# Plachtaa/FAcodec

Measured on NVIDIA H100. Metric: audio_seconds_per_second, higher is better.
Workload: dtype f32 I/O and accumulation; every product is a 3-MMA split of fp32 operands: fp16 hi + 2^11-scaled fp16 lo (22 mantissa bits, register-promoted accumulation) upstream of the VQ, bf16 hi + bf16 lo (16 bits) downstream

## Files before the change

### facodec_b200/_lib.py

```python
import ctypes
import os

from . import build as _build

_c = ctypes
_LIB = None


class FacError(RuntimeError):
    pass


def lib_path():
    return _build.LIB


def load():
    global _LIB
    if _LIB is not None:
        return _LIB
    path = lib_path()
    if not os.path.exists(path):
        raise FacError(f"{path} not found: build it with `python -m facodec_b200.build` "
                       "(needs nvcc; there is no CPU fallback)")
    L = ctypes.CDLL(path)
    vp, i32, i64p, fp = _c.c_void_p, _c.c_int, _c.c_void_p, _c.c_void_p
    sigs = {
        "fac_abi_version": ([], i32),
        "fac_create": ([_c.POINTER(vp), i32], i32),
        "fac_destroy": ([vp], i32),
        "fac_last_error": ([vp], _c.c_char_p),
        "fac_load_tensor": ([vp, i32, _c.c_char_p, fp, _c.POINTER(_c.c_int64), i32], i32),
        "fac_finalize": ([vp], i32),
        "fac_encode": ([vp, fp, i32, i32, fp, vp], i32),
        "fac_encode_frames": ([i32], i32),
        "fac_quantize": ([vp, fp, fp, i32, i32, i32, i32, fp, i32, i64p, fp, fp, fp, fp, fp, fp, i64p, i64p, i64p, vp], i32),
        "fac_decode": ([vp, fp, i32, i32, fp, vp], i32),
        "fac_codec_forward": ([vp, fp, i32, i32, i32, fp, i64p, i64p, i64p, fp, vp], i32),
        "fac_codec_forward_host": ([vp, fp, i32, i32, i32, fp, i64p, i64p, i64p, vp], i32),
        "fac_codec_encode": ([vp, fp, i32, i32, i32, i64p, i64p, i64p, fp, vp], i32),
        "fac_dequantize": ([vp, i64p, i64p, i32, i64p, i32, fp, i32, i32, fp, fp, fp, fp, vp], i32),
        "fac_codes_decode": ([vp, i64p, i64p, i32, i64p, i32, fp, i32, i32, fp, vp], i32),
        "fac_redecode": ([vp, i64p, i64p, i32, fp, i32, i32, i32, i32, i32, fp, vp], i32),
        "fac_redecoder_decode": ([vp, fp, i32, i32, fp, vp], i32),
        "fac_voice_convert": ([vp, i64p, i64p, i32, fp, i32, i32, i32, i32, i32, fp, vp], i32),
        "fac_dataset_mel": ([vp, fp, i32, i32, fp, vp], i32),
        "fac_head_begin": ([vp], i32),
        "fac_head_tensor": ([vp, i32, _c.c_char_p, fp, _c.POINTER(_c.c_int64), i32], i32),
        "fac_head_finalize": ([vp, i32, i32, i32, i32, i32], i32),
        "fac_head_forward": ([vp, i32, fp, i32, i32, _c.POINTER(vp), vp], i32),
        "fac_rvq_create": ([vp, i32] + [_c.POINTER(vp)] * 5, i32),
        "fac_rvq_destroy": ([vp, i32], i32),
        "fac_stream_begin": ([vp, i32], i32),
        "fac_stream_encode": ([vp, i32, fp, i32, fp, vp], i32),
        "fac_stream_decode": ([vp, i32, fp, i32, fp, vp], i32),
        "fac_stream_decode_codes": ([vp, i32, i64p, i64p, i32, i64p, i32, fp, i32, fp, vp], i32),
        "fac_stream_encode_codes": ([vp, i32, fp, i32, i32, i64p, i64p, i64p, vp], i32),
        "fac_stream_finish_codes": ([vp, i32, i64p, i64p, i64p, fp, vp], i32),
        "fac_stream_end": ([vp, i32], i32),
        "fac_spectral_loss": ([vp, fp, fp, i32, i32, i32, i32, _c.POINTER(_c.c_int), _c.POINTER(_c.c_int), fp, fp,
                               _c.c_float, _c.c_float, _c.c_float, _c.c_float, fp, vp], i32),
        "fac_l1_loss": ([vp, fp, fp, _c.c_longlong, fp, vp], i32),
        "fac_add3": ([vp, fp, fp, fp, _c.c_longlong, fp, vp], i32),
        "fac_reconstruction_loss": ([vp, fp, fp, i32, i32, fp, fp, vp], i32),
        "fac_rvq_forward": ([vp, i32, fp, i32, i32, i32, fp, i64p, fp, vp], i32),
        "fac_alias_free_act": ([vp, fp, i32, i32, i32, i32, fp, fp, fp, vp], i32),
        "fac_debug_conv": ([vp, fp, fp, fp] + [i32] * 10 + [fp, fp, i32, fp, fp, i32, vp], i32),
        "fac_debug_conv_tc": ([vp, fp, fp, fp] + [i32] * 10 + [fp, fp, i32, fp, fp, i32, i32, vp], i32),
        "fac_debug_resunit": ([vp, fp, fp, fp, fp, fp, fp, fp, i32, i32, i32, i32, i32, fp, vp], i32),
        "fac_debug_tc_phase_clocks": ([vp, _c.POINTER(_c.c_longlong)], i32),
        "fac_debug_tc_producer_clocks": ([vp, _c.POINTER(_c.c_longlong)], i32),
        "fac_debug_tc_trace": ([vp, _c.POINTER(_c.c_longlong)], i32),
        "fac_debug_lstm_pack": ([fp, i32, i32, fp, _c.c_longlong, _c.POINTER(_c.c_int)], _c.c_longlong),
        "fac_debug_convtr_pack": ([fp, i32, i32, i32, i32, fp, _c.c_longlong], _c.c_longlong),
        "fac_debug_pad_map": ([i32, i32, i32, i32, _c.POINTER(_c.c_int), i32], i32),
        "fac_debug_tc_plan": ([i32] * 8 + [_c.POINTER(_c.c_int)], i32),
        "fac_debug_tc_pack": ([fp, i32, i32, i32, i32, i32, fp, _c.c_longlong], _c.c_longlong),
        "fac_debug_lstm_phase_clocks": ([vp, _c.POINTER(_c.c_longlong)], i32),
        "fac_set_option": ([vp, _c.c_char_p, i32], i32),
        "fac_debug_slstm": ([vp, fp, _c.POINTER(vp), i32, i32, i32, fp, vp], i32),
        "fac_debug_fa_quantize": ([vp, fp, fp, _c.POINTER(vp), fp, i32, i32, i32, i32, i32, fp, fp, fp, fp, i64p, i64p, i64p,
                                   fp, fp, vp], i32),
        "fac_debug_attention": ([vp, fp, fp, fp, fp, i32, i32, i32, _c.c_void_p, i32, vp], i32),
        "fac_debug_tap": ([vp, _c.c_char_p, fp, _c.c_size_t], i32),
        "fac_profile_enable": ([vp, i32], i32),
        "fac_profile_reset": ([vp], i32),
        "fac_profile_get": ([vp, _c.c_char_p, _c.POINTER(_c.c_double), _c.POINTER(_c.c_double),
                             _c.POINTER(_c.c_double), _c.POINTER(_c.c_longlong)], i32),
        "fac_profile_dump": ([vp, _c.c_char_p, _c.c_size_t], _c.c_size_t),
        "fac_workspace_bytes": ([vp], _c.c_size_t),
        "fac_last_launch_count": ([vp], i32),
    }
    for name, (args, res) in sigs.items():
        fn = getattr(L, name)
        fn.argtypes = args
        fn.restype = res
    _LIB = L
    return L


EXPORTED = ["fac_abi_version", "fac_create", "fac_destroy", "fac_last_error", "fac_load_tensor", "fac_finalize",
            "fac_encode", "fac_encode_frames", "fac_quantize", "fac_decode", "fac_codec_forward",
            "fac_codec_forward_host", "fac_codec_encode", "fac_dequantize", "fac_codes_decode", "fac_redecode", "fac_redecoder_decode", "fac_voice_convert", "fac_dataset_mel", "fac_reconstruction_loss", "fac_spectral_loss", "fac_l1_loss", "fac_head_begin", "fac_head_tensor", "fac_head_finalize", "fac_head_forward", "fac_add3", "fac_stream_begin", "fac_stream_encode", "fac_stream_decode", "fac_stream_decode_codes", "fac_stream_encode_codes", "fac_stream_finish_codes", "fac_stream_end", "fac_rvq_create", "fac_rvq_destroy", "fac_rvq_forward", "fac_alias_free_act",
            "fac_debug_conv", "fac_debug_conv_tc", "fac_debug_resunit", "fac_debug_tc_phase_clocks", "fac_debug_tc_producer_clocks", "fac_debug_tc_trace", "fac_debug_lstm_pack", "fac_debug_convtr_pack", "fac_debug_pad_map", "fac_debug_tc_plan", "fac_debug_tc_pack", "fac_debug_lstm_phase_clocks", "fac_set_option", "fac_debug_slstm", "fac_debug_fa_quantize", "fac_debug_attention", "fac_debug_tap", "fac_profile_enable", "fac_profile_reset", "fac_profile_get", "fac_profile_dump",
            "fac_workspace_bytes", "fac_last_launch_count"]


def check(handle, rc, what):
    if rc < 0:
        msg = load().fac_last_error(handle)
        raise FacError(f"{what} failed (status {rc}): {msg.decode() if msg else ''}")
    return rc
```

### facodec_b200/csrc/conv_tc.cu

```cuda
#include <cuda_bf16.h>
#include <cuda_fp16.h>

#include <cstring>
#include <mutex>

#include "common.cuh"
#include "conv_tc_common.cuh"
#include "kernels.h"

namespace fac {

namespace {

using namespace tc;

enum Prec { P_TF32 = 0, P_BF16 = 1, P_F16S = 2, P_F16X2 = 3, P_NONE = -1 };

template <int P> struct PrecT {
    static constexpr int KG = P == P_TF32 ? 4 : 2;
    static constexpr int planes = P == P_F16S ? 1 : 2;
    static constexpr int ksteps = P == P_TF32 ? 2 : 1;
    static constexpr int kind = P == P_TF32 ? WG_TF32 : (P == P_BF16 ? WG_BF16 : WG_F16);
};

__host__ __device__ constexpr int prec_kg(int P) { return P == P_TF32 ? 4 : 2; }
__host__ __device__ constexpr int prec_planes(int P) { return P == P_F16S ? 1 : 2; }
__host__ __device__ constexpr uint32_t master_bytes(bool promoted, int nchunk, int promote_every, int ni) {
    return promoted && nchunk > promote_every ? (uint32_t)ni / 2 * 4 * kThreads : 0u;
}

template <int NI>
__device__ __forceinline__ void zero_acc(float (&a)[NI / 2]) {
#pragma unroll
    for (int i = 0; i < NI / 2; ++i) a[i] = 0.f;
}

template <int P, int NI>
__device__ __forceinline__ void mma_pass(float (&acc)[NI / 2], uint32_t a_addr, uint32_t a_lbo, uint32_t b_addr,
                                         uint32_t b_lbo) {
#pragma unroll
    for (int ks = 0; ks < PrecT<P>::ksteps; ++ks)
        wgmma_ss<NI, PrecT<P>::kind>(acc, gdesc(a_addr + ks * 2 * a_lbo, a_lbo, 128), gdesc(b_addr + ks * 2 * b_lbo, b_lbo, 128));
}

struct Tile {
    int row0, col0, nw;
    int warp, lane;
};

template <int NI, int GROUP = NI, typename F>
__device__ __forceinline__ void for_each_pair(const Tile& tl, const float (&acc)[NI / 2], F&& f) {
#pragma unroll
    for (int j = 0; j < NI / 8; ++j) {
        if (j > 0 && (8 * j) % GROUP == 0 && 8 * j >= tl.nw) break;
#pragma unroll
        for (int h = 0; h < 2; ++h) {
            const int row = tl.row0 + 16 * tl.warp + (tl.lane >> 2) + 8 * h;
            const int col = tl.col0 + 8 * j + 2 * (tl.lane & 3);
            f(row, col, acc[4 * j + 2 * h], acc[4 * j + 2 * h + 1]);
        }
    }
}

template <bool FAST>
__device__ __forceinline__ float act_out(int act, float v, float al, float ia) {
    if (act == ACT_SNAKE) return FAST ? fmaf(ia, sin2_mufu(al * v), v) : snake_fast(v, al, ia);
    if (act == ACT_TANH) return tanhf(v);
    if (act == ACT_MISH) return mish_f(v);
    return v;
}

template <int P1, int P2, bool PROMO, int NI, int MINB = 1, bool TT = false>
__global__ void __launch_bounds__(kThreads, MINB) conv_tc_kernel(TcConvParams p) {
    constexpr bool FUSED = P2 != P_NONE;
    static_assert(!TT || (NI == 64 && !FUSED), "transposed tiles: <= 64 channels x 64 time steps per warpgroup");
    static_assert(NI % 16 == 0 && NI <= (PROMO || MINB == 2 ? 64 : (P1 == P_F16S ? 256 : 128)),
                  "accumulator registers: <= 64 / 128 columns (256 in the one-pass fp16 class at one CTA per SM)");
    constexpr bool F16X2 = P1 == P_F16X2;
    constexpr bool DEC = P1 == P_BF16 || P1 == P_F16S;
    using T1 = PrecT<P1>;
    extern __shared__ __align__(1024) uint8_t smem[];
    uint64_t* full = reinterpret_cast<uint64_t*>(smem);

    const int tid = threadIdx.x, wg = tid >> 7;
    const int BM = 64 * p.MT;
    const int N = p.N, NW = p.MT == 2 ? N : N / 2;
    Tile tl;
    tl.row0 = p.MT == 2 ? 64 * wg : 0;
    tl.col0 = p.MT == 2 ? 0 : wg * NW;
    tl.nw = NW;
    tl.warp = (tid >> 5) & 3;
    tl.lane = tid & 31;
    const int t0 = blockIdx.x * BM, ntile = blockIdx.y, b = blockIdx.z;
    const int Kr = p.Kr, dil = p.dil, Rpad = p.Rpad, nchunk = p.nchunk, S = p.stagesB;
    const int R = BM + (Kr - 1) * dil;
    const uint32_t a_plane = (uint32_t)T1::KG * Rpad * 16, a_bytes = a_plane * T1::planes;
    uint8_t* abuf = smem + kSmemHdr;
    float4* master = reinterpret_cast<float4*>(abuf + 2 * (size_t)a_bytes);
    uint8_t* wbuf = abuf + 2 * (size_t)a_bytes + master_bytes(PROMO, nchunk, p.promote_every, NI);
    uint8_t* a2buf = wbuf + (size_t)S * p.b_slot;
    const uint32_t w_unit1 = (uint32_t)Kr * T1::planes * T1::KG * N * 16;
    const uint32_t w_unit2 = FUSED ? (uint32_t)prec_planes(P2) * prec_kg(P2) * N * 16 : 0;
    const int units = nchunk + (FUSED ? p.nchunk2 : 0);

    if (tid == 0) {
        for (int i = 0; i < S; ++i) mbar_init(&full[i], 1);
        fence_mbar_init();
    }
    __syncthreads();
    auto issue_w = [&](int u) {
        uint64_t* bar = &full[u % S];
        uint8_t* dst = wbuf + (size_t)(u % S) * p.b_slot;
        const uint8_t* src;
        uint32_t bytes;
        if (u < nchunk) { src = reinterpret_cast<const uint8_t*>(p.wblob) + ((size_t)ntile * nchunk + u) * w_unit1; bytes = w_unit1; }
        else { src = reinterpret_cast<const uint8_t*>(p.wblob2) + (size_t)(u - nchunk) * w_unit2; bytes = w_unit2; }
        mbar_arrive_expect_tx(bar, bytes);
        bulk_g2s(dst, src, bytes, bar);
    };
    if (tid == 0)
        for (int u = 0; u < S - 1 && u < units; ++u) issue_w(u);

    const PadMap pm = PadMap::make(p.Tin, p.pad_left_s, p.pad_right_s, p.reflect);
    const float* __restrict__ xb = p.x + (size_t)b * p.x_bstride;
    auto produce = [&](int c) {
        uint8_t* ahi = abuf + (size_t)(c & 1) * a_bytes;
        if constexpr (P1 == P_TF32) produce_chunk<kThreads, false>(p, pm, xb, c, t0, R, Rpad, ahi, ahi + a_plane, tid);
        else if constexpr (P1 == P_BF16) produce_chunk<kThreads, true>(p, pm, xb, c, t0, R, Rpad, ahi, ahi + a_plane, tid);
        else if constexpr (P1 == P_F16S) produce_chunk<kThreads, true, 4, false, false, true>(p, pm, xb, c, t0, R, Rpad, ahi, ahi, tid);
        else produce_chunk<kThreads, false, 4, false, true>(p, pm, xb, c, t0, R, Rpad, ahi, ahi + a_plane, tid);
        fence_proxy_async();
    };
    produce(0);

    float acc[NI / 2];
    float crs[F16X2 ? NI / 2 : 1];
    zero_acc<NI>(acc);
    if constexpr (F16X2) zero_acc<NI>(crs);
    const uint32_t a_lbo = (uint32_t)Rpad * 16, b_lbo = (uint32_t)N * 16;
    const uint32_t abase = smem_u32(abuf), wbase = smem_u32(wbuf), a2base = smem_u32(a2buf);
    const int BM2 = BM;

    auto promote = [&](bool first, bool last) {
        if constexpr (PROMO) {
#pragma unroll
            for (int q = 0; q < NI / 8; ++q) {
                float w[4];
#pragma unroll
                for (int e = 0; e < 4; ++e) {
                    const int i = 4 * q + e;
                    if constexpr (F16X2) { w[e] = acc[i] + crs[i] * kLoUnscale; crs[i] = 0.f; }
                    else w[e] = acc[i];
                }
                float4 m = first ? make_float4(0.f, 0.f, 0.f, 0.f) : master[q * kThreads + tid];
                m.x += w[0]; m.y += w[1]; m.z += w[2]; m.w += w[3];
                if (!last) master[q * kThreads + tid] = m;
                acc[4 * q + 0] = last ? m.x : 0.f;
                acc[4 * q + 1] = last ? m.y : 0.f;
                acc[4 * q + 2] = last ? m.z : 0.f;
                acc[4 * q + 3] = last ? m.w : 0.f;
            }
        }
    };

#pragma unroll 1
    for (int u = 0; u < units; ++u) {
        __syncthreads();
        if (tid == 0 && u + S - 1 < units) issue_w(u + S - 1);
        mbar_wait(&full[u % S], (uint32_t)(u / S) & 1u);
        const uint32_t wslot = wbase + (uint32_t)(u % S) * p.b_slot;
        wg_fence();
        if (u < nchunk) {
            const uint32_t a0 = abase + (uint32_t)(u & 1) * a_bytes + (uint32_t)tl.row0 * 16;
            const uint32_t b0 = wslot + (uint32_t)tl.col0 * 16;
#pragma unroll 1
            for (int tap = 0; tap < Kr; ++tap) {
                const uint32_t ahi = a0 + (uint32_t)(tap * dil) * 16, alo = ahi + a_plane;
                const uint32_t bhi = b0 + (uint32_t)tap * T1::planes * T1::KG * b_lbo, blo = bhi + T1::KG * b_lbo;
                if constexpr (TT) {
                    mma_pass<P1, NI>(acc, bhi, b_lbo, ahi, a_lbo);
                    mma_pass<P1, NI>(crs, bhi, b_lbo, alo, a_lbo);
                    mma_pass<P1, NI>(crs, blo, b_lbo, ahi, a_lbo);
                } else if constexpr (P1 == P_F16S) {
                    mma_pass<P1, NI>(acc, ahi, a_lbo, bhi, b_lbo);
                } else if constexpr (F16X2) {
// ... 81 lines not shown
    for_each_pair<NI>(tl, acc, [&](int row, int col, float v0, float v1) {
        const int t = t0 + row;
        if (t >= p.Tout) return;
        if (bi_p) { const float2 bi = __ldg(reinterpret_cast<const float2*>(bi_p + col)); v0 += bi.x; v1 += bi.y; }
        if (act == ACT_SNAKE) {
            const float2 al = __ldg(reinterpret_cast<const float2*>(al_p + col));
            const float2 ia = __ldg(reinterpret_cast<const float2*>(ia_p + col));
            v0 = act_out<DEC>(ACT_SNAKE, v0, al.x, ia.x);
            v1 = act_out<DEC>(ACT_SNAKE, v1, al.y, ia.y);
        } else if (act != ACT_NONE) {
            v0 = act_out<DEC>(act, v0, 0.f, 0.f);
            v1 = act_out<DEC>(act, v1, 0.f, 0.f);
        }
        if (rb) { const float2 r = *reinterpret_cast<const float2*>(rb + (size_t)t * p.ldy + col); v0 += r.x; v1 += r.y; }
        *reinterpret_cast<float2*>(yb + (size_t)t * p.ldy + col) = make_float2(v0, v1);
    });
}

}

namespace {
constexpr size_t kSmemCap = 227 * 1024;
constexpr size_t kSmemCap2 = 113 * 1024;
int plan_prec(const TcConvParams& p) {
    return p.g1f16 ? P_F16S : (p.f16x2 ? P_F16X2 : (p.bf16 ? P_BF16 : P_TF32));
}
constexpr int f16s_wide_nw(bool fused) { return fused ? 192 : 256; }
}

bool tc_conv_plan(TcConvParams& p) {
    if ((p.Cin % 4) != 0 || ((p.Cin * p.vf) % kChunk) != 0 || (p.Cout % 16) != 0) return false;
    if (p.bf16 && p.promoted) return false;
    if (p.f16x2 && !p.promoted) return false;
    if (p.g1f16 && !p.bf16) return false;
    if (p.tt && !p.f16x2) return false;
    if (p.fused && (p.promoted || p.Cin != p.Cout || p.vf != 1 || p.Cout > 256)) return false;
    const int P1 = plan_prec(p), P2 = p.fused ? (p.bf16 ? P_BF16 : P_TF32) : P_NONE;
    p.nchunk = p.Cin * p.vf / kChunk;
    p.nchunk2 = p.fused ? p.Cout / kChunk : 0;
    p.promote_every = p.promoted ? (p.f16x2 ? (48 / p.Kr < 1 ? 1 : 48 / p.Kr) : (8 / p.Kr < 1 ? 1 : 8 / p.Kr)) : 1;
    const int nw_max = p.promoted ? 64 : 128;
    constexpr size_t kAReserve = 40 * 1024;
    int N = 0;
    for (int cand = p.fused ? p.Cout : 256; cand >= 16 && N == 0; cand -= 16) {
        const bool rows_split = cand <= nw_max, cols_split = (cand / 2) % 16 == 0 && cand / 2 <= nw_max;
        if (p.Cout % cand || !(rows_split || cols_split)) continue;
        size_t slot = (size_t)p.Kr * prec_planes(P1) * prec_kg(P1) * cand * 16, a2 = 0;
        if (P2 != P_NONE) a2 = (size_t)prec_planes(P2) * p.nchunk2 * prec_kg(P2) * 64 * 16;
        if (kSmemHdr + kAReserve + slot + a2 <= kSmemCap) N = cand;
        else if (p.fused) return false;
    }
    if (N == 0) return false;
    struct Layout { int Rpad; size_t slot, total; };
    auto layout = [&](int S, int MT) {
        const int NW = MT == 2 ? N : N / 2, BM = 64 * MT;
        Layout l;
        l.Rpad = BM + (p.Kr - 1) * p.dil;
        while (l.Rpad % 8 != 2) ++l.Rpad;
        const size_t a_bytes = (size_t)prec_planes(P1) * prec_kg(P1) * l.Rpad * 16;
        l.slot = (size_t)p.Kr * prec_planes(P1) * prec_kg(P1) * N * 16;
        size_t a2 = 0;
        if (P2 != P_NONE) {
            const size_t slot2 = (size_t)prec_planes(P2) * prec_kg(P2) * N * 16;
            if (slot2 > l.slot) l.slot = slot2;
            a2 = (size_t)prec_planes(P2) * p.nchunk2 * prec_kg(P2) * BM * 16;
        }
        const size_t master = master_bytes(p.promoted, p.nchunk, p.promote_every, p.tt ? 64 : NW);
        l.total = kSmemHdr + 2 * a_bytes + master + S * l.slot + a2 + (p.tt ? 64 * 16 : 0);
        return l;
    };
    const bool want2 = p.promoted ? !p.tt : (p.occ2_maxn > 0 && N <= p.occ2_maxn);
    for (int two = want2 ? 1 : 0; two >= 0; --two) {
        const size_t cap = two ? kSmemCap2 : kSmemCap;
        const int nwl = two ? 64 : nw_max;
        for (int S = 2; S >= 1; --S)
            for (int MT = 2; MT >= 1; --MT) {
                const int NW = MT == 2 ? N : N / 2;
                const bool wide = !two && P1 == P_F16S && NW == f16s_wide_nw(p.fused);
                if ((NW > nwl && !wide) || NW % 16) continue;
                if (wide && layout(2, 1).total <= kSmemCap2) continue;
                const Layout l = layout(S, MT);
                if (l.total > cap) continue;
                p.N = N; p.MT = MT; p.Rpad = l.Rpad; p.R2pad = 64 * MT; p.stagesB = S; p.b_slot = (int)l.slot;
                p.smem_bytes = l.total;
                p.occ2 = two;
                return true;
            }
    }
    return false;
}

size_t tc_blob_floats(const TcConvParams& p) {
    if (p.g1f16) return (size_t)(p.Cout / p.N) * p.nchunk * p.Kr * 2 * p.N * 4;
    return (size_t)(p.Cout / p.N) * p.nchunk * p.Kr * 2 * ((p.bf16 || p.f16x2) ? 2 : 4) * p.N * 4;
}

static inline uint16_t bf16_rn_host(float f) {
    uint32_t u;
    memcpy(&u, &f, 4);
    u += 0x7FFFu + ((u >> 16) & 1u);
    return (uint16_t)(u >> 16);
}

void tc_pack_blob(const TcConvParams& p, const float* wp, int ldw, float* blob) {
    const int Cw = p.Cin * p.vf;
    if (p.g1f16) {
        uint16_t* ob = reinterpret_cast<uint16_t*>(blob);
        size_t o16 = 0;
        for (int nt = 0; nt < p.Cout / p.N; ++nt)
            for (int c = 0; c < p.nchunk; ++c)
                for (int tap = 0; tap < p.Kr; ++tap)
                    for (int k8 = 0; k8 < 2; ++k8)
                        for (int n = 0; n < p.N; ++n)
                            for (int e = 0; e < 8; ++e) {
                                int kk = tap * Cw + c * tc::kChunk + k8 * 8 + e;
                                __half v = __float2half_rn(wp[(size_t)kk * ldw + nt * p.N + n]);
                                uint16_t bits;
                                memcpy(&bits, &v, 2);
                                ob[o16++] = bits;
                            }
        return;
    }
    if (p.f16x2) {
        uint16_t* ob = reinterpret_cast<uint16_t*>(blob);
        size_t o16 = 0;
        for (int nt = 0; nt < p.Cout / p.N; ++nt)
            for (int c = 0; c < p.nchunk; ++c)
                for (int tap = 0; tap < p.Kr; ++tap)
                    for (int hl = 0; hl < 2; ++hl)
                        for (int k8 = 0; k8 < 2; ++k8)
                            for (int n = 0; n < p.N; ++n)
                                for (int e = 0; e < 8; ++e) {
                                    int kk = tap * Cw + c * tc::kChunk + k8 * 8 + e;
                                    float w = wp[(size_t)kk * ldw + nt * p.N + n];
                                    __half hi = __float2half_rn(w);
                                    __half v = hl == 0 ? hi : __float2half_rn((w - __half2float(hi)) * 2048.0f);
// ... 111 lines not shown
```

### facodec_b200/csrc/conv_tc_common.cuh

```cuda
#pragma once
#include <cuda_bf16.h>
#include <cuda_fp16.h>

#include "common.cuh"
#include "kernels.h"

namespace fac {

namespace tc {

constexpr int kThreads = 256;
constexpr int kChunk = 16;
constexpr int kSmemHdr = 128;

__device__ __forceinline__ uint32_t smem_u32(const void* p) { return (uint32_t)__cvta_generic_to_shared(p); }

__device__ __forceinline__ void mbar_init(uint64_t* bar, uint32_t count) {
    asm volatile("mbarrier.init.shared::cta.b64 [%0], %1;" ::"r"(smem_u32(bar)), "r"(count));
}
__device__ __forceinline__ void mbar_arrive(uint64_t* bar) {
    asm volatile("mbarrier.arrive.shared::cta.b64 _, [%0];" ::"r"(smem_u32(bar)) : "memory");
}
__device__ __forceinline__ void mbar_arrive_expect_tx(uint64_t* bar, uint32_t bytes) {
    asm volatile("mbarrier.arrive.expect_tx.shared::cta.b64 _, [%0], %1;" ::"r"(smem_u32(bar)), "r"(bytes) : "memory");
// ... 156 lines not shown
    uint32_t r;
    asm("cvt.rna.tf32.f32 %0, %1;" : "=r"(r) : "f"(x));
    return __uint_as_float(r);
}


template <bool BF16>
__device__ __forceinline__ void split_store(float4 x4, int pc, int row, int Rpad, uint8_t* ahi, uint8_t* alo) {
    if constexpr (!BF16) {
        float4 hi, lo;
        hi.x = to_tf32(x4.x); lo.x = to_tf32(x4.x - hi.x);
        hi.y = to_tf32(x4.y); lo.y = to_tf32(x4.y - hi.y);
        hi.z = to_tf32(x4.z); lo.z = to_tf32(x4.z - hi.z);
        hi.w = to_tf32(x4.w); lo.w = to_tf32(x4.w - hi.w);
        const size_t off = ((size_t)pc * Rpad + row) * 16;
        *reinterpret_cast<float4*>(ahi + off) = hi;
        *reinterpret_cast<float4*>(alo + off) = lo;
    } else {
        __nv_bfloat162 h01 = __floats2bfloat162_rn(x4.x, x4.y), h23 = __floats2bfloat162_rn(x4.z, x4.w);
        float2 f01 = __bfloat1622float2(h01), f23 = __bfloat1622float2(h23);
        __nv_bfloat162 l01 = __floats2bfloat162_rn(x4.x - f01.x, x4.y - f01.y);
        __nv_bfloat162 l23 = __floats2bfloat162_rn(x4.z - f23.x, x4.w - f23.y);
        const size_t off = ((size_t)(pc >> 1) * Rpad + row) * 16 + (size_t)(pc & 1) * 8;
        uint2 hv, lv;
        hv.x = *reinterpret_cast<uint32_t*>(&h01); hv.y = *reinterpret_cast<uint32_t*>(&h23);
        lv.x = *reinterpret_cast<uint32_t*>(&l01); lv.y = *reinterpret_cast<uint32_t*>(&l23);
        *reinterpret_cast<uint2*>(ahi + off) = hv;
        *reinterpret_cast<uint2*>(alo + off) = lv;
    }
}

constexpr float kLoScale = 2048.0f, kLoUnscale = 1.0f / 2048.0f;
__device__ __forceinline__ void split_store_f16(float4 x4, int pc, int row, int Rpad, uint8_t* ahi, uint8_t* alo) {
    __half2 h01 = __floats2half2_rn(x4.x, x4.y), h23 = __floats2half2_rn(x4.z, x4.w);
    float2 f01 = __half22float2(h01), f23 = __half22float2(h23);
    __half2 l01 = __floats2half2_rn((x4.x - f01.x) * kLoScale, (x4.y - f01.y) * kLoScale);
    __half2 l23 = __floats2half2_rn((x4.z - f23.x) * kLoScale, (x4.w - f23.y) * kLoScale);
    const size_t off = ((size_t)(pc >> 1) * Rpad + row) * 16 + (size_t)(pc & 1) * 8;
    uint2 hv, lv;
    hv.x = *reinterpret_cast<uint32_t*>(&h01); hv.y = *reinterpret_cast<uint32_t*>(&h23);
    lv.x = *reinterpret_cast<uint32_t*>(&l01); lv.y = *reinterpret_cast<uint32_t*>(&l23);
    *reinterpret_cast<uint2*>(ahi + off) = hv;
    *reinterpret_cast<uint2*>(alo + off) = lv;
}

__device__ __forceinline__ void store_f16_single(float4 x4, int pc, int row, int Rpad, uint8_t* ahi) {
    __half2 h01 = __floats2half2_rn(x4.x, x4.y), h23 = __floats2half2_rn(x4.z, x4.w);
    const size_t off = ((size_t)(pc >> 1) * Rpad + row) * 16 + (size_t)(pc & 1) * 8;
    uint2 hv;
    hv.x = *reinterpret_cast<uint32_t*>(&h01); hv.y = *reinterpret_cast<uint32_t*>(&h23);
    *reinterpret_cast<uint2*>(ahi + off) = hv;
}

template <int NT, bool BF16, int BATCH = 4, bool INL = false, bool F16 = false, bool SINGLE = false>
__device__ __forceinline__ void produce_chunk(const TcConvParams& p, const PadMap& pm, const float* __restrict__ xb,
                                              int c, int t0, int R, int Rpad, uint8_t* ahi, uint8_t* alo, int ptid) {
    const int pc = ptid & 3;
    const int j = c * kChunk + pc * 4;
    const int soff = j / p.Cin, ci = j - soff * p.Cin;
    const bool has_alpha = p.in_alpha != nullptr;
    float4 al = make_float4(0.f, 0.f, 0.f, 0.f), ia = al;
    if (has_alpha) {
        al = __ldg(reinterpret_cast<const float4*>(p.in_alpha + ci));
        ia = __ldg(reinterpret_cast<const float4*>(p.in_inv_alpha + ci));
    }
    constexpr int RSTEP = NT / 4;
    const int row_limit = p.Tout + (p.Kr - 1) * p.dil;
    const int vrow0 = t0 - p.PLr;
    const float* __restrict__ xcol = xb + ci;
#pragma unroll 1
    for (int r = ptid >> 2; r < R; r += RSTEP * BATCH) {
        float4 v[BATCH];
#pragma unroll
        for (int u = 0; u < BATCH; ++u) {
            const int rr = r + u * RSTEP;
            v[u] = make_float4(0.f, 0.f, 0.f, 0.f);
            const int vrow = vrow0 + rr;
            if (rr < R && vrow < row_limit) {
                const int src = pm.src(vrow * p.vf + soff);
                if (src >= 0) v[u] = __ldg(reinterpret_cast<const float4*>(xcol + (size_t)src * p.ldx));
            }
        }
#pragma unroll
        for (int u = 0; u < BATCH; ++u) {
            const int rr = r + u * RSTEP;
            if (rr < R) {
                float4 x4 = v[u];
                if (has_alpha) x4 = snake4_sel<BF16, INL>(x4, al, ia);
                if constexpr (SINGLE) store_f16_single(x4, pc, rr, Rpad, ahi);
                else if constexpr (F16) split_store_f16(x4, pc, rr, Rpad, ahi, alo);
                else split_store<BF16>(x4, pc, rr, Rpad, ahi, alo);
            }
        }
    }
}

}

}
```

### facodec_b200/csrc/engine.cu

```cuda
#include <cmath>
#include <cstdio>
#include <cstdlib>
#include <cstring>
#include <map>
#include <string>
#include <vector>

#include "../../include/facodec_b200.h"
#include "../../include/facodec_b200_debug.h"
#include "common.cuh"
#include "kernels.h"

using namespace fac;

namespace {

constexpr int HOP = 300;
constexpr int LATENT = 1024;
constexpr int N_FFT = 2048;
constexpr int WIN = 1200;
constexpr int N_BINS = 1025;
constexpr int SPEC_LD = 2052;
constexpr int SPEC_TC_LD = 2176;
constexpr int N_MELS = 80;
// ... 2564 lines not shown
    for (int i = 0; i < 8; ++i) {
        HostTensor t;
        const bool mat = (i % 4) < 2;
        if (mat) t.shape = {4 * H, H}; else t.shape = {4 * H};
        if (i == 1) t.data.assign(whh_host, whh_host + (size_t)4 * H * H);
        else t.data.assign(t.numel(), 0.f);
        tmp.host[0][std::string("l.") + names[i]] = std::move(t);
    }
    LstmW L;
    try { L = pack_lstm(&tmp, 0, "l"); } catch (const PackError&) { return FAC_ERR_UNSUPPORTED; }
    if (info3) { info3[0] = L.U; info3[1] = L.G; info3[2] = 4 * L.U; }
    if (bf16 == 2 || bf16 == 3) {
        const int p3 = bf16 == 3;
        const long long n2 = (long long)lstm2_pack_words(H, L.U, p3);
        if (!out || capacity_floats < n2) return n2;
        lstm2_pack(whh_host, H, L.U, p3, reinterpret_cast<uint32_t*>(out));
        return n2;
    }
    const long long n = (long long)L.G * H * 4 * L.U;
    if (bf16 && !L.has16) return FAC_ERR_UNSUPPORTED;
    if (!out || capacity_floats < n) return n;
    memcpy(out, tmp.pack.data() + (bf16 ? L.whh16[0] : L.whh[0]), sizeof(float) * (size_t)n);
    return n;
}

long long fac_debug_convtr_pack(const float* w_host, int Cin, int Cout, int stride, int causal, float* out, long long capacity_floats) {
    if (!w_host || Cin <= 0 || Cout <= 0 || stride <= 0) return FAC_ERR_INVALID;
    fac_handle tmp;
    HostTensor t, b;
    t.shape = {Cin, Cout, 2 * stride};
    t.data.assign(w_host, w_host + (size_t)Cin * Cout * 2 * stride);
    b.shape = {Cout};
    b.data.assign(Cout, 0.f);
    tmp.host[0]["c.weight"] = std::move(t);
    tmp.host[0]["c.bias"] = std::move(b);
    ConvW c;
    try { c = causal ? pack_convtr(&tmp, 0, "c", stride) : pack_convtr_noncausal(&tmp, 0, "c", stride); }
    catch (const PackError&) { return FAC_ERR_UNSUPPORTED; }
    const long long n = (long long)c.K * Cin * c.Cout;
    if (!out || capacity_floats < n) return n;
    for (int k = 0; k < c.K; ++k)
        for (int ci = 0; ci < Cin; ++ci)
            for (int co = 0; co < c.Cout; ++co) out[((size_t)k * Cin + ci) * c.Cout + co] = tmp.pack[c.w + ((size_t)k * Cin + ci) * c.ldw + co];
    return n;
}

int fac_debug_pad_map(int L, int pad_left, int pad_right, int reflect, int* out, int n) {
    if (!out || L < 0 || pad_left < 0 || pad_right < 0 || n != pad_left + L + pad_right) return FAC_ERR_INVALID;
    const PadMap pm = PadMap::make(L, pad_left, pad_right, reflect);
    for (int i = 0; i < n; ++i) out[i] = pm.src(i - pad_left);
    return FAC_OK;
}

int fac_debug_tc_plan(int Cin, int Cout, int K, int dil, int stride, int Tout, int mode, int occ2_maxn, int* out8) {
    if (!out8 || Cin <= 0 || Cout <= 0 || K <= 0 || dil <= 0 || stride <= 0 || mode < 0 || mode > 8) return FAC_ERR_INVALID;
    TcConvParams tp;
    tp.Cin = Cin; tp.Cout = Cout; tp.Tout = Tout; tp.occ2_maxn = occ2_maxn;
    tp.promoted = (mode == 1 || mode == 3) ? 1 : 0;
    tp.bf16 = (mode == 2 || mode == 4 || mode == 7 || mode == 8) ? 1 : 0;
    tp.f16x2 = mode == 3 ? 1 : 0;
    tp.fused = (mode == 4 || mode == 5 || mode == 8) ? 1 : 0;
    tp.g1f16 = (mode == 7 || mode == 8) ? 1 : 0;
    if (mode == 6) { tp.promoted = 1; tp.f16x2 = 1; tp.tt = 1; }
    if (stride == 1) { tp.vf = 1; tp.Kr = K; tp.dil = dil; }
    else if (K == 2 * stride && dil == 1) { tp.vf = stride; tp.Kr = 2; tp.dil = 1; }
    else return FAC_ERR_UNSUPPORTED;
    if (!tc_conv_plan(tp)) return FAC_ERR_UNSUPPORTED;
    out8[0] = tp.N; out8[1] = tp.MT; out8[2] = tp.nchunk; out8[3] = tp.stagesB; out8[4] = tp.R2pad;
    out8[5] = (int)tp.smem_bytes; out8[6] = tp.Rpad; out8[7] = tp.promote_every;
    return FAC_OK;
}

long long fac_debug_tc_pack(const float* w_host, int Cin, int Cout, int K, int stride, int mode, float* blob_out,
                            long long capacity_floats) {
    if (!w_host || Cin <= 0 || Cout <= 0 || K <= 0 || stride <= 0 || mode < 0 || mode > 3) return FAC_ERR_INVALID;
    TcConvParams tp;
    tp.Cin = Cin; tp.Cout = Cout; tp.dil = 1;
    tp.promoted = (mode == 1 || mode == 3) ? 1 : 0; tp.bf16 = mode == 2 ? 1 : 0; tp.f16x2 = mode == 3 ? 1 : 0;
    if (stride == 1) { tp.vf = 1; tp.Kr = K; }
    else if (K == 2 * stride) { tp.vf = stride; tp.Kr = 2; }
    else return FAC_ERR_UNSUPPORTED;
    if (!tc_conv_plan(tp)) return FAC_ERR_UNSUPPORTED;
    const long long n = (long long)tc_blob_floats(tp);
    if (!blob_out || capacity_floats < n) return n;
    const int ldw = (Cout + 3) / 4 * 4;
    std::vector<float> gen((size_t)K * Cin * ldw, 0.f);
    for (int co = 0; co < Cout; ++co)
        for (int ci = 0; ci < Cin; ++ci)
            for (int k = 0; k < K; ++k) gen[((size_t)k * Cin + ci) * ldw + co] = w_host[((size_t)co * Cin + ci) * K + k];
    tc_pack_blob(tp, gen.data(), ldw, blob_out);
    return n;
}

int fac_debug_tc_phase_clocks(fac_handle* h, long long* out8) {
    if (!h || !out8) return FAC_ERR_INVALID;
    h->err = "fac_debug_tc_phase_clocks: the tensor-core conv kernel records no timing probes";
    return FAC_ERR_UNSUPPORTED;
}

int fac_debug_tc_trace(fac_handle* h, long long* out80) {
    if (!h || !out80) return FAC_ERR_INVALID;
    h->err = "fac_debug_tc_trace: the tensor-core conv kernel records no timing probes";
    return FAC_ERR_UNSUPPORTED;
}

int fac_debug_tc_producer_clocks(fac_handle* h, long long* out4) {
    if (!h || !out4) return FAC_ERR_INVALID;
    h->err = "fac_debug_tc_producer_clocks: the tensor-core conv kernel records no timing probes";
    return FAC_ERR_UNSUPPORTED;
}

int fac_debug_lstm_phase_clocks(fac_handle* h, long long* out4) {
    if (!h || !out4) return FAC_ERR_INVALID;
    cudaSetDevice(h->device);
    cudaDeviceSynchronize();
    cudaError_t e = h->lstm_v2 ? lstm2_read_phase_clocks(out4) : lstm_read_phase_clocks(out4);
    if (e != cudaSuccess) { h->err = cudaGetErrorString(e); return FAC_ERR_CUDA; }
    return FAC_OK;
}

int fac_debug_tap(fac_handle* h, const char* name, float* dst, size_t capacity_floats) {
    if (!h || !name) return FAC_ERR_INVALID;
    if (!dst) h->taps.erase(name);
// ... 71 lines not shown
```

### facodec_b200/csrc/kernels.h

```cpp
#pragma once
#include <cuda_runtime.h>
#include <stdint.h>

namespace fac {

struct ConvParams {
    const float* x = nullptr;
    const float* w = nullptr;
    const float* bias = nullptr;
    const float* in_alpha = nullptr;
    const float* in_inv_alpha = nullptr;
    const float* out_alpha = nullptr;
    const float* out_inv_alpha = nullptr;
    const float* res = nullptr;
    const int* valid_len = nullptr;
    float* y = nullptr;
    int B = 0, Tin = 0, Cin = 0, Tout = 0, Cout = 0;
    int K = 1, dil = 1, stride = 1, pad_left = 0, pad_right = 0, pad_reflect = 0;
    int ldw = 0, ldy = 0, ldx = 0;
    int out_act = 0;
    int y_transposed = 0;
    size_t x_bstride = 0, y_bstride = 0;
};
cudaError_t launch_conv(const ConvParams& p, cudaStream_t st);

struct TcConvParams {
    const float* x = nullptr;
    const float* wblob = nullptr;
    const float* bias = nullptr;
    const float* in_alpha = nullptr;
    const float* in_inv_alpha = nullptr;
    const float* out_alpha = nullptr;
    const float* out_inv_alpha = nullptr;
    const float* res = nullptr;
    float* y = nullptr;
    int B = 0, Tin = 0, Cin = 0, ldx = 0;
    int vf = 1;
    int Kr = 1, dil = 1, PLr = 0;
    int pad_left_s = 0, pad_right_s = 0, reflect = 0;
    int Tout = 0, Cout = 0, ldy = 0;
    int out_act = 0;
    int promoted = 0;
    int bf16 = 0;
    int g1f16 = 0;
    int f16x2 = 0;
    int fused = 0;
    int tt = 0;
    int occ2_maxn = 0;
    const float* wblob2 = nullptr;
    const float* bias2 = nullptr;
    int nchunk2 = 0;
    int promote_every = 1;
    int N = 0, nchunk = 0, Rpad = 0, stagesB = 0;
    int MT = 2;
    int b_slot = 0;
    int occ2 = 0;
    int R2pad = 0;
    size_t smem_bytes = 0;
    size_t x_bstride = 0, y_bstride = 0;
};
bool tc_conv_plan(TcConvParams& p);
size_t tc_blob_floats(const TcConvParams& p);
void tc_pack_blob(const TcConvParams& p, const float* wp, int ldw, float* blob);
cudaError_t launch_conv_tc(const TcConvParams& p, cudaStream_t st);

struct LstmParams {
    const float* xg = nullptr;
    const float* whh_p = nullptr;
    const float* whh_p16 = nullptr;
    int bf16 = 0;
    const uint32_t* whh_p2 = nullptr;
    uint32_t* h16 = nullptr;
    int pass3 = 0;
    uint32_t* state_h = nullptr;
    float* state_c = nullptr;
    const float* skip = nullptr;
    float* y = nullptr;
    float* hT = nullptr;
    unsigned int* bar = nullptr;
    int B = 0, T = 0, H = 0, U = 0, G = 0;
};
cudaError_t launch_lstm_layer(const LstmParams& p, cudaStream_t st);
cudaError_t launch_lstm2_layer(const LstmParams& p, cudaStream_t st);
size_t lstm2_pack_words(int H, int U, int pass3);
void lstm2_pack(const float* whh, int H, int U, int pass3, uint32_t* out);
size_t lstm2_smem_bytes(int H, int U, int pass3);
cudaError_t lstm2_read_phase_clocks(long long* out4);
int lstm_units_per_cta(int H);
cudaError_t lstm_read_phase_clocks(long long* out4);

cudaError_t launch_stft_frames(const float* wave, float* frames , int B, int T, int F, int hop, int win, int pad,
                               cudaStream_t st, int f_first = 0);
cudaError_t launch_mel_from_spec(const float* spec, int ldspec, const float* fb , float* mel,
                                 int B, int F, int Tm, cudaStream_t st);

struct VqWeights {
    const float* w_in;
    const float* b_in;
    const float* cb;
    const float* cbn;
    const float* cbn2;
    const float* w_out;
    const float* b_out;
};
struct FaqParams {
    const float* f0 = nullptr;
// ... 64 lines not shown
```

### include/facodec_b200_debug.h

```cpp
#ifndef FACODEC_B200_DEBUG_H
#define FACODEC_B200_DEBUG_H

#include "facodec_b200.h"

#ifdef __cplusplus
extern "C" {
#endif

int fac_debug_conv(fac_handle* h, const float* x, const float* w_host, const float* bias_host, int B, int Tin,
                   int Cin, int Cout, int K, int dil, int stride, int pad_left, int pad_right, int reflect,
                   const float* in_alpha_host, const float* out_alpha_host, int act, const float* res,
                   float* y, int Tout, void* stream);
int fac_debug_conv_tc(fac_handle* h, const float* x, const float* w_host, const float* bias_host, int B, int Tin,
                      int Cin, int Cout, int K, int dil, int stride, int pad_left, int pad_right, int reflect,
                      const float* in_alpha_host, const float* out_alpha_host, int act, const float* res,
                      float* y, int Tout, int promoted, void* stream);
int fac_debug_resunit(fac_handle* h, const float* x, const float* w7_host, const float* b7_host, const float* w1_host,
                      const float* b1_host, const float* alpha1_host, const float* alpha2_host, int B, int T, int C,
                      int dil, int mode, float* y, void* stream);
int fac_debug_tc_phase_clocks(fac_handle* h, long long* out8);
int fac_debug_tc_producer_clocks(fac_handle* h, long long* out4);
int fac_debug_tc_trace(fac_handle* h, long long* out80);
long long fac_debug_lstm_pack(const float* whh_host, int H, int bf16, float* out, long long capacity_floats, int* info3);
int fac_debug_pad_map(int L, int pad_left, int pad_right, int reflect, int* out, int n);
int fac_debug_tc_plan(int Cin, int Cout, int K, int dil, int stride, int Tout, int mode, int occ2_maxn, int* out8);
long long fac_debug_tc_pack(const float* w_host, int Cin, int Cout, int K, int stride, int mode, float* blob_out,
                            long long capacity_floats);
int fac_debug_lstm_phase_clocks(fac_handle* h, long long* out4);
long long fac_debug_convtr_pack(const float* w_host, int Cin, int Cout, int stride, int causal, float* out,
                                long long capacity_floats);
int fac_debug_slstm(fac_handle* h, const float* x, const float* const* w_host, int B, int T, int H, float* y,
                    void* stream);
int fac_debug_fa_quantize(fac_handle* h, const float* f0, const float* z, const float* const vq_host[6][5],
                          const float* gamma_beta, int n_c, int B, int Tq, int Tz, int Tf0, float* outs, float* zp,
                          float* zc, float* zr, int64_t* codes_p, int64_t* codes_c, int64_t* codes_r, float* sqerr,
                          float* losses2, void* stream);
int fac_debug_attention(fac_handle* h, const float* q, const float* k, const float* v, float* o, int B, int T,
                        int heads, const int* valid_len, int force_stream, void* stream);
int fac_debug_tap(fac_handle* h, const char* name, float* dst, size_t capacity_floats);

int fac_profile_enable(fac_handle* h, int on);
int fac_profile_reset(fac_handle* h);
int fac_profile_get(fac_handle* h, const char* family, double* ms, double* flops, double* bytes,
                    long long* launches);
size_t fac_profile_dump(fac_handle* h, char* buf, size_t cap);

#ifdef __cplusplus
}
#endif
#endif
```

Baseline: 923.7.

## Stage next activation chunk via cp.async while converting current chunk

Adds an optional staging buffer, reusing the second-stage A region when it fits, that prefetches the next input chunk from global memory with cp.async. The producer then converts the staged fp32 data into split hi/lo tiles from shared memory instead of loading from global directly. The planner turns staging on when the extra shared memory fits the budget. The launch bounds also change to request two blocks per SM whenever NI <= 128, which caps register use and may cause spills. The INL snake template option is removed.

Result: faster. 969.9 (median of 6 runs) (+5.0%).

```diff
diff --git a/facodec_b200/_lib.py b/facodec_b200/_lib.py
--- a/facodec_b200/_lib.py
+++ b/facodec_b200/_lib.py
@@ -75,6 +75,7 @@
         "fac_debug_convtr_pack": ([fp, i32, i32, i32, i32, fp, _c.c_longlong], _c.c_longlong),
         "fac_debug_pad_map": ([i32, i32, i32, i32, _c.POINTER(_c.c_int), i32], i32),
         "fac_debug_tc_plan": ([i32] * 8 + [_c.POINTER(_c.c_int)], i32),
+        "fac_debug_tc_staged": ([i32] * 8, i32),
         "fac_debug_tc_pack": ([fp, i32, i32, i32, i32, i32, fp, _c.c_longlong], _c.c_longlong),
         "fac_debug_lstm_phase_clocks": ([vp, _c.POINTER(_c.c_longlong)], i32),
         "fac_set_option": ([vp, _c.c_char_p, i32], i32),
@@ -102,7 +103,7 @@
 EXPORTED = ["fac_abi_version", "fac_create", "fac_destroy", "fac_last_error", "fac_load_tensor", "fac_finalize",
             "fac_encode", "fac_encode_frames", "fac_quantize", "fac_decode", "fac_codec_forward",
             "fac_codec_forward_host", "fac_codec_encode", "fac_dequantize", "fac_codes_decode", "fac_redecode", "fac_redecoder_decode", "fac_voice_convert", "fac_dataset_mel", "fac_reconstruction_loss", "fac_spectral_loss", "fac_l1_loss", "fac_head_begin", "fac_head_tensor", "fac_head_finalize", "fac_head_forward", "fac_add3", "fac_stream_begin", "fac_stream_encode", "fac_stream_decode", "fac_stream_decode_codes", "fac_stream_encode_codes", "fac_stream_finish_codes", "fac_stream_end", "fac_rvq_create", "fac_rvq_destroy", "fac_rvq_forward", "fac_alias_free_act",
-            "fac_debug_conv", "fac_debug_conv_tc", "fac_debug_resunit", "fac_debug_tc_phase_clocks", "fac_debug_tc_producer_clocks", "fac_debug_tc_trace", "fac_debug_lstm_pack", "fac_debug_convtr_pack", "fac_debug_pad_map", "fac_debug_tc_plan", "fac_debug_tc_pack", "fac_debug_lstm_phase_clocks", "fac_set_option", "fac_debug_slstm", "fac_debug_fa_quantize", "fac_debug_attention", "fac_debug_tap", "fac_profile_enable", "fac_profile_reset", "fac_profile_get", "fac_profile_dump",
+            "fac_debug_conv", "fac_debug_conv_tc", "fac_debug_resunit", "fac_debug_tc_phase_clocks", "fac_debug_tc_producer_clocks", "fac_debug_tc_trace", "fac_debug_lstm_pack", "fac_debug_convtr_pack", "fac_debug_pad_map", "fac_debug_tc_plan", "fac_debug_tc_staged", "fac_debug_tc_pack", "fac_debug_lstm_phase_clocks", "fac_set_option", "fac_debug_slstm", "fac_debug_fa_quantize", "fac_debug_attention", "fac_debug_tap", "fac_profile_enable", "fac_profile_reset", "fac_profile_get", "fac_profile_dump",
             "fac_workspace_bytes", "fac_last_launch_count"]
 
 
diff --git a/facodec_b200/csrc/conv_tc.cu b/facodec_b200/csrc/conv_tc.cu
--- a/facodec_b200/csrc/conv_tc.cu
+++ b/facodec_b200/csrc/conv_tc.cu
@@ -71,7 +71,7 @@
 }
 
 template <int P1, int P2, bool PROMO, int NI, int MINB = 1, bool TT = false>
-__global__ void __launch_bounds__(kThreads, MINB) conv_tc_kernel(TcConvParams p) {
+__global__ void __launch_bounds__(kThreads, NI <= 128 ? 2 : MINB) conv_tc_kernel(TcConvParams p) {
     constexpr bool FUSED = P2 != P_NONE;
     static_assert(!TT || (NI == 64 && !FUSED), "transposed tiles: <= 64 channels x 64 time steps per warpgroup");
     static_assert(NI % 16 == 0 && NI <= (PROMO || MINB == 2 ? 64 : (P1 == P_F16S ? 256 : 128)),
@@ -99,6 +99,7 @@
     float4* master = reinterpret_cast<float4*>(abuf + 2 * (size_t)a_bytes);
     uint8_t* wbuf = abuf + 2 * (size_t)a_bytes + master_bytes(PROMO, nchunk, p.promote_every, NI);
     uint8_t* a2buf = wbuf + (size_t)S * p.b_slot;
+    uint8_t* stage = p.stage_act ? a2buf : nullptr;
     const uint32_t w_unit1 = (uint32_t)Kr * T1::planes * T1::KG * N * 16;
     const uint32_t w_unit2 = FUSED ? (uint32_t)prec_planes(P2) * prec_kg(P2) * N * 16 : 0;
     const int units = nchunk + (FUSED ? p.nchunk2 : 0);
@@ -123,14 +124,30 @@
 
     const PadMap pm = PadMap::make(p.Tin, p.pad_left_s, p.pad_right_s, p.reflect);
     const float* __restrict__ xb = p.x + (size_t)b * p.x_bstride;
+    auto stage_next = [&](int c) {
+        if (c < nchunk) {
+            stage_chunk<kThreads>(p, pm, xb, c, t0, R, smem_u32(stage), tid);
+            cp_async_commit();
+        }
+    };
     auto produce = [&](int c) {
         uint8_t* ahi = abuf + (size_t)(c & 1) * a_bytes;
-        if constexpr (P1 == P_TF32) produce_chunk<kThreads, false>(p, pm, xb, c, t0, R, Rpad, ahi, ahi + a_plane, tid);
-        else if constexpr (P1 == P_BF16) produce_chunk<kThreads, true>(p, pm, xb, c, t0, R, Rpad, ahi, ahi + a_plane, tid);
-        else if constexpr (P1 == P_F16S) produce_chunk<kThreads, true, 4, false, false, true>(p, pm, xb, c, t0, R, Rpad, ahi, ahi, tid);
-        else produce_chunk<kThreads, false, 4, false, true>(p, pm, xb, c, t0, R, Rpad, ahi, ahi + a_plane, tid);
+        if (stage) {
+            cp_async_wait_all();
+            if constexpr (P1 == P_TF32) consume_chunk<kThreads, false>(p, c, R, Rpad, stage, ahi, ahi + a_plane, tid);
+            else if constexpr (P1 == P_BF16) consume_chunk<kThreads, true>(p, c, R, Rpad, stage, ahi, ahi + a_plane, tid);
+            else if constexpr (P1 == P_F16S) consume_chunk<kThreads, true, false, true>(p, c, R, Rpad, stage, ahi, ahi, tid);
+            else consume_chunk<kThreads, false, true>(p, c, R, Rpad, stage, ahi, ahi + a_plane, tid);
+            stage_next(c + 1);
+        } else {
+            if constexpr (P1 == P_TF32) produce_chunk<kThreads, false>(p, pm, xb, c, t0, R, Rpad, ahi, ahi + a_plane, tid);
+            else if constexpr (P1 == P_BF16) produce_chunk<kThreads, true>(p, pm, xb, c, t0, R, Rpad, ahi, ahi + a_plane, tid);
+            else if constexpr (P1 == P_F16S) produce_chunk<kThreads, true, 4, false, true>(p, pm, xb, c, t0, R, Rpad, ahi, ahi, tid);
+            else produce_chunk<kThreads, false, 4, true>(p, pm, xb, c, t0, R, Rpad, ahi, ahi + a_plane, tid);
+        }
         fence_proxy_async();
     };
+    if (stage) stage_next(0);
     produce(0);
 
     float acc[NI / 2];
@@ -318,10 +335,11 @@
     }
     if (N == 0) return false;
     struct Layout { int Rpad; size_t slot, total; };
-    auto layout = [&](int S, int MT) {
+    auto layout = [&](int S, int MT, bool staged) {
         const int NW = MT == 2 ? N : N / 2, BM = 64 * MT;
         Layout l;
-        l.Rpad = BM + (p.Kr - 1) * p.dil;
+        const int R = BM + (p.Kr - 1) * p.dil;
+        l.Rpad = R;
         while (l.Rpad % 8 != 2) ++l.Rpad;
         const size_t a_bytes = (size_t)prec_planes(P1) * prec_kg(P1) * l.Rpad * 16;
         l.slot = (size_t)p.Kr * prec_planes(P1) * prec_kg(P1) * N * 16;
@@ -332,8 +350,14 @@
             a2 = (size_t)prec_planes(P2) * p.nchunk2 * prec_kg(P2) * BM * 16;
         }
         const size_t master = master_bytes(p.promoted, p.nchunk, p.promote_every, p.tt ? 64 : NW);
-        l.total = kSmemHdr + 2 * a_bytes + master + S * l.slot + a2 + (p.tt ? 64 * 16 : 0);
+        const size_t stage = staged ? stage_slot_bytes(R) : 0;
+        l.total = kSmemHdr + 2 * a_bytes + master + S * l.slot + (a2 > stage ? a2 : stage) + (p.tt ? 64 * 16 : 0);
         return l;
+    };
+    auto staged = [&](int S, int MT, size_t cap) {
+        if (p.Kr != 1 && MT != 2) return false;
+        const size_t budget = layout(S, MT, false).total <= kSmemCap2 ? kSmemCap2 : cap;
+        return layout(S, MT, true).total <= budget;
     };
     const bool want2 = p.promoted ? !p.tt : (p.occ2_maxn > 0 && N <= p.occ2_maxn);
     for (int two = want2 ? 1 : 0; two >= 0; --two) {
@@ -344,10 +368,11 @@
                 const int NW = MT == 2 ? N : N / 2;
                 const bool wide = !two && P1 == P_F16S && NW == f16s_wide_nw(p.fused);
                 if ((NW > nwl && !wide) || NW % 16) continue;
-                if (wide && layout(2, 1).total <= kSmemCap2) continue;
-                const Layout l = layout(S, MT);
-                if (l.total > cap) continue;
-                p.N = N; p.MT = MT; p.Rpad = l.Rpad; p.R2pad = 64 * MT; p.stagesB = S; p.b_slot = (int)l.slot;
+                if (wide && layout(2, 1, false).total <= kSmemCap2) continue;
+                if (layout(S, MT, false).total > cap) continue;
+                const bool st = staged(S, MT, cap);
+                const Layout l = layout(S, MT, st);
+                p.N = N; p.MT = MT; p.Rpad = l.Rpad; p.R2pad = 64 * MT; p.stagesB = S; p.stage_act = st; p.b_slot = (int)l.slot;
                 p.smem_bytes = l.total;
                 p.occ2 = two;
                 return true;
diff --git a/facodec_b200/csrc/conv_tc_common.cuh b/facodec_b200/csrc/conv_tc_common.cuh
--- a/facodec_b200/csrc/conv_tc_common.cuh
+++ b/facodec_b200/csrc/conv_tc_common.cuh
@@ -232,7 +232,31 @@
     *reinterpret_cast<uint2*>(ahi + off) = hv;
 }
 
-template <int NT, bool BF16, int BATCH = 4, bool INL = false, bool F16 = false, bool SINGLE = false>
+__host__ __device__ constexpr uint32_t stage_slot_bytes(int R) { return ((uint32_t)R * 64 + 127) & ~127u; }
+
+__device__ __forceinline__ void cp_async16(uint32_t dst, const void* src, uint32_t src_bytes) {
+    asm volatile("cp.async.cg.shared.global [%0], [%1], 16, %2;" ::"r"(dst), "l"(src), "r"(src_bytes) : "memory");
+}
+__device__ __forceinline__ void cp_async_commit() { asm volatile("cp.async.commit_group;" ::: "memory"); }
+__device__ __forceinline__ void cp_async_wait_all() { asm volatile("cp.async.wait_group 0;" ::: "memory"); }
+
+template <int NT>
+__device__ __forceinline__ void stage_chunk(const TcConvParams& p, const PadMap& pm, const float* __restrict__ xb, int c,
+                                            int t0, int R, uint32_t slot, int ptid) {
+    const int pc = ptid & 3;
+    const int j = c * kChunk + pc * 4;
+    const int soff = j / p.Cin, ci = j - soff * p.Cin;
+    const int row_limit = p.Tout + (p.Kr - 1) * p.dil;
+    const int vrow0 = t0 - p.PLr;
+    const float* __restrict__ xcol = xb + ci;
+    for (int rr = ptid >> 2; rr < R; rr += NT / 4) {
+        const int vrow = vrow0 + rr;
+        const int src = vrow < row_limit ? pm.src(vrow * p.vf + soff) : -1;
+        cp_async16(slot + (uint32_t)rr * 64 + pc * 16, xcol + (size_t)(src < 0 ? 0 : src) * p.ldx, src < 0 ? 0u : 16u);
+    }
+}
+
+template <int NT, bool BF16, int BATCH = 4, bool F16 = false, bool SINGLE = false>
 __device__ __forceinline__ void produce_chunk(const TcConvParams& p, const PadMap& pm, const float* __restrict__ xb,
                                               int c, int t0, int R, int Rpad, uint8_t* ahi, uint8_t* alo, int ptid) {
     const int pc = ptid & 3;
@@ -266,7 +290,7 @@
             const int rr = r + u * RSTEP;
             if (rr < R) {
                 float4 x4 = v[u];
-                if (has_alpha) x4 = snake4_sel<BF16, INL>(x4, al, ia);
+                if (has_alpha) x4 = snake4_sel<BF16>(x4, al, ia);
                 if constexpr (SINGLE) store_f16_single(x4, pc, rr, Rpad, ahi);
                 else if constexpr (F16) split_store_f16(x4, pc, rr, Rpad, ahi, alo);
                 else split_store<BF16>(x4, pc, rr, Rpad, ahi, alo);
@@ -275,6 +299,26 @@
     }
 }
 
-}
-
-}
+template <int NT, bool BF16, bool F16 = false, bool SINGLE = false>
+__device__ __forceinline__ void consume_chunk(const TcConvParams& p, int c, int R, int Rpad, const uint8_t* slot,
+                                              uint8_t* ahi, uint8_t* alo, int ptid) {
+    const int pc = ptid & 3;
+    const int ci = (c * kChunk + pc * 4) % p.Cin;
+    const bool has_alpha = p.in_alpha != nullptr;
+    float4 al = make_float4(0.f, 0.f, 0.f, 0.f), ia = al;
+    if (has_alpha) {
+        al = __ldg(reinterpret_cast<const float4*>(p.in_alpha + ci));
+        ia = __ldg(reinterpret_cast<const float4*>(p.in_inv_alpha + ci));
+    }
+    for (int rr = ptid >> 2; rr < R; rr += NT / 4) {
+        float4 x4 = *reinterpret_cast<const float4*>(slot + (size_t)rr * 64 + pc * 16);
+        if (has_alpha) x4 = snake4_sel<BF16>(x4, al, ia);
+        if constexpr (SINGLE) store_f16_single(x4, pc, rr, Rpad, ahi);
+        else if constexpr (F16) split_store_f16(x4, pc, rr, Rpad, ahi, alo);
+        else split_store<BF16>(x4, pc, rr, Rpad, ahi, alo);
+    }
+}
+
+}
+
+}
diff --git a/facodec_b200/csrc/engine.cu b/facodec_b200/csrc/engine.cu
--- a/facodec_b200/csrc/engine.cu
+++ b/facodec_b200/csrc/engine.cu
@@ -2640,9 +2640,8 @@
     return FAC_OK;
 }
 
-int fac_debug_tc_plan(int Cin, int Cout, int K, int dil, int stride, int Tout, int mode, int occ2_maxn, int* out8) {
-    if (!out8 || Cin <= 0 || Cout <= 0 || K <= 0 || dil <= 0 || stride <= 0 || mode < 0 || mode > 8) return FAC_ERR_INVALID;
-    TcConvParams tp;
+static int debug_tc_plan(int Cin, int Cout, int K, int dil, int stride, int Tout, int mode, int occ2_maxn, TcConvParams& tp) {
+    if (Cin <= 0 || Cout <= 0 || K <= 0 || dil <= 0 || stride <= 0 || mode < 0 || mode > 8) return FAC_ERR_INVALID;
     tp.Cin = Cin; tp.Cout = Cout; tp.Tout = Tout; tp.occ2_maxn = occ2_maxn;
     tp.promoted = (mode == 1 || mode == 3) ? 1 : 0;
     tp.bf16 = (mode == 2 || mode == 4 || mode == 7 || mode == 8) ? 1 : 0;
@@ -2653,10 +2652,23 @@
     if (stride == 1) { tp.vf = 1; tp.Kr = K; tp.dil = dil; }
     else if (K == 2 * stride && dil == 1) { tp.vf = stride; tp.Kr = 2; tp.dil = 1; }
     else return FAC_ERR_UNSUPPORTED;
-    if (!tc_conv_plan(tp)) return FAC_ERR_UNSUPPORTED;
+    return tc_conv_plan(tp) ? FAC_OK : FAC_ERR_UNSUPPORTED;
+}
+
+int fac_debug_tc_plan(int Cin, int Cout, int K, int dil, int stride, int Tout, int mode, int occ2_maxn, int* out8) {
+    if (!out8) return FAC_ERR_INVALID;
+    TcConvParams tp;
+    const int rc = debug_tc_plan(Cin, Cout, K, dil, stride, Tout, mode, occ2_maxn, tp);
+    if (rc != FAC_OK) return rc;
     out8[0] = tp.N; out8[1] = tp.MT; out8[2] = tp.nchunk; out8[3] = tp.stagesB; out8[4] = tp.R2pad;
     out8[5] = (int)tp.smem_bytes; out8[6] = tp.Rpad; out8[7] = tp.promote_every;
     return FAC_OK;
+}
+
+int fac_debug_tc_staged(int Cin, int Cout, int K, int dil, int stride, int Tout, int mode, int occ2_maxn) {
+    TcConvParams tp;
+    const int rc = debug_tc_plan(Cin, Cout, K, dil, stride, Tout, mode, occ2_maxn, tp);
+    return rc != FAC_OK ? rc : tp.stage_act;
 }
 
 long long fac_debug_tc_pack(const float* w_host, int Cin, int Cout, int K, int stride, int mode, float* blob_out,
diff --git a/facodec_b200/csrc/kernels.h b/facodec_b200/csrc/kernels.h
--- a/facodec_b200/csrc/kernels.h
+++ b/facodec_b200/csrc/kernels.h
@@ -52,6 +52,7 @@
     int nchunk2 = 0;
     int promote_every = 1;
     int N = 0, nchunk = 0, Rpad = 0, stagesB = 0;
+    int stage_act = 0;
     int MT = 2;
     int b_slot = 0;
     int occ2 = 0;
diff --git a/include/facodec_b200_debug.h b/include/facodec_b200_debug.h
--- a/include/facodec_b200_debug.h
+++ b/include/facodec_b200_debug.h
@@ -24,6 +24,7 @@
 long long fac_debug_lstm_pack(const float* whh_host, int H, int bf16, float* out, long long capacity_floats, int* info3);
 int fac_debug_pad_map(int L, int pad_left, int pad_right, int reflect, int* out, int n);
 int fac_debug_tc_plan(int Cin, int Cout, int K, int dil, int stride, int Tout, int mode, int occ2_maxn, int* out8);
+int fac_debug_tc_staged(int Cin, int Cout, int K, int dil, int stride, int Tout, int mode, int occ2_maxn);
 long long fac_debug_tc_pack(const float* w_host, int Cin, int Cout, int K, int stride, int mode, float* blob_out,
                             long long capacity_floats);
 int fac_debug_lstm_phase_clocks(fac_handle* h, long long* out4);
```
